# adamnelsonarcher/BB-OCR

Hardware: AMD Instinct MI355X
Metric: book-page images/sec end-to-end (detect+recognize) @1280x960 (higher is better)
Workload: dtype fp16

## Files before the change

bb-ocr_amd/csrc/conv_mfma.hip:

```cpp
#include "common.h"
#include "kernels.h"
#include <type_traits>
#include <utility>

template <int EL, int MF, bool ADDUP = false>
__device__ __forceinline__ void conv_epilogue(const ConvArgs& a, f32x4 (&acc)[MF][4], int n, int nt, int oy0, int ox0, int wm, int wn, int fpr,
                                              int lane, int BN, int sub = 1, int sph = 0, int spw = 0) {
    const int g = lane >> 4, pl = lane & 15;
    const int cout0 = nt * BN + wn * 64 + g * 8;
    if (a.tail) {
        const float* tw = a.tail;
        const typename El<EL>::v8 w1f = *(const typename El<EL>::v8*)(a.tail_frag + lane * 8);
        float cb[8], b1r[4], w2a[4], w2b[4];
#pragma unroll
        for (int i = 0; i < 8; ++i) cb[i] = a.bias[(g & 1) * 8 + i];
#pragma unroll
        for (int r = 0; r < 4; ++r) { b1r[r] = tw[4 * g + r]; w2a[r] = tw[16 + 4 * g + r]; w2b[r] = tw[32 + 4 * g + r]; }
        const float b20 = tw[48], b21 = tw[49];
#pragma unroll
        for (int f = 0; f < MF; ++f) {
            const int F = wm * MF + f;
            const int fr = F / fpr, fc = F - fr * fpr;
            const int oy = (oy0 + fr) * sub + sph, ox = (ox0 + fc * 16 + pl) * sub + spw;
            u32x4 bb;
#pragma unroll
            for (int j = 0; j < 2; ++j) {
                const float x0 = fmaxf(acc[f][j][0] + cb[j * 4 + 0], 0.f), x1 = fmaxf(acc[f][j][1] + cb[j * 4 + 1], 0.f);
                const float x2 = fmaxf(acc[f][j][2] + cb[j * 4 + 2], 0.f), x3 = fmaxf(acc[f][j][3] + cb[j * 4 + 3], 0.f);
// ... 62 lines not shown
            pack_runs(v, lo, hi);
            uint16_t* op = (uint16_t*)base + row + (size_t)x * cs + cout0 + coff;
            *(u32x4*)(op) = lo;
            if (run1) *(u32x4*)(op + 32) = hi;
        }
    };
    auto split_hi_lo = [&](const float (&v)[16], float (&vh)[16], float (&vl)[16]) {
#pragma unroll
        for (int i = 0; i < 16; ++i) {
            vh[i] = El<EL>::to_f32(El<EL>::from_f32(v[i]));
            vl[i] = (v[i] - vh[i]) * SPLIT_LO_SCALE;
        }
    };
    auto store_frag = [&](void* base, size_t row, int cs, int xb, int xlim, bool row_ok, const float (&v)[16], bool f32) {
        if (a.split_off) {
            float vh[16], vl[16];
            split_hi_lo(v, vh, vl);
            store_frag_at(base, row, cs, xb, xlim, row_ok, vh, false, 0);
            store_frag_at(base, row, cs, xb, xlim, row_ok, vl, false, a.split_off);
            return;
        }
        store_frag_at(base, row, cs, xb, xlim, row_ok, v, f32, 0);
    };
    if constexpr (ADDUP) {
        struct Gather { u32x4 q[8]; f32x2_t w[4]; };
        const int hw = a.up_H * a.up_W, LH = a.up_H >> 1, LW = a.up_W >> 1;
        const float rhw = 1.f / (float)hw, rw = 1.f / (float)a.up_W;
        auto issue = [&](int f, Gather& G) {
            int p = ox0 + (wm * MF + f) * 16 + pl;
            p = p < a.OW ? p : a.OW - 1;
            int ni = (int)((float)p * rhw);
            int rem = p - ni * hw;
            if (rem < 0) { --ni; rem += hw; } else if (rem >= hw) { ++ni; rem -= hw; }
            int yy = (int)((float)rem * rw);
            int xx = rem - yy * a.up_W;
            if (xx < 0) { --yy; xx += a.up_W; } else if (xx >= a.up_W) { ++yy; xx -= a.up_W; }
            float sy = ((float)yy + 0.5f) * 0.5f - 0.5f, sx = ((float)xx + 0.5f) * 0.5f - 0.5f;
            sy = sy < 0.f ? 0.f : sy;
            sx = sx < 0.f ? 0.f : sx;
            const int y0 = (int)sy, x0 = (int)sx;
            const int y1 = y0 + (y0 < LH - 1 ? 1 : 0), x1 = x0 + (x0 < LW - 1 ? 1 : 0);
            const float ly = sy - (float)y0, lx = sx - (float)x0, hy = 1.f - ly, hx = 1.f - lx;
            G.w[0] = (f32x2_t){hy * hx, hy * hx}; G.w[1] = (f32x2_t){hy * lx, hy * lx};
            G.w[2] = (f32x2_t){ly * hx, ly * hx}; G.w[3] = (f32x2_t){ly * lx, ly * lx};
            const uint16_t* zb = a.addup + (size_t)ni * LH * LW * a.up_cs + cout0;
            const uint16_t* z00 = zb + ((size_t)y0 * LW + x0) * a.up_cs;
            const uint16_t* z01 = zb + ((size_t)y0 * LW + x1) * a.up_cs;
// ... 1066 lines not shown
    const size_t smem = 18 * 2048 + 2 * 324 * 64 + 256;
    static LdsOptIn attr;
    if (hipError_t e = lds_opt_in(attr, (const void*)conv3x3_up4_kernel<EL>, smem); e != hipSuccess) return e;
    const int grid = ntiles < 2 * ncu ? ntiles : 2 * ncu;
    hipLaunchKernelGGL(conv3x3_up4_kernel<EL>, dim3(grid), dim3(256), smem, s, a);
    return hipGetLastError();
}

hipError_t launch_up4_fused(const ConvPlan& p1, const ConvPlan& p3, ConvArgs a, hipStream_t s) {
    if (p1.KH != 1 || p1.Cin != 128 || p1.Cout != 64 || p1.BN != 64 || p3.KH != 3 || p3.Cin != 64 || p3.Cout_pad != 64 || p3.BN != 64 ||
        p1.el != p3.el || p1.split || p3.split || a.in0_cs != 128 || a.up_cs != 64 || !a.addup || !a.zero || a.cout_store > 32 || (a.up_H & 1) || (a.up_W & 1) ||
        a.up_H != a.H || a.up_W != a.W)
        return hipErrorNotSupported;
    a.KH = a.KW = 3; a.pad_h = a.pad_w = 1; a.dil = 1; a.sub = 1;
    a.OH = a.H; a.OW = a.W; a.TH = a.TW = 16;
    a.tiles_x = (a.OW + 15) / 16; a.tiles_y = (a.OH + 15) / 16; a.ntiles_n = 1; a.nchunks = 2; a.ntaps = 9;
    a.aux_w = p1.d_w; a.aux_b = p1.d_b;
    a.wpk = p3.d_w; a.bias = p3.d_b;
    a.acc_scale = 1.f;
    if ((long long)a.N * a.tiles_x * a.tiles_y > 0x7fffffffLL) return hipErrorNotSupported;
    return p3.el ? launch_up4_el<1>(a, s) : launch_up4_el<0>(a, s);
}

template <int EL, int WM, int WN, int MF, int RING, bool ADDUP>
__global__ void __launch_bounds__(WM * WN * 64, (WM * WN == 8 ? 1 : 2)) conv1x1_dma_kernel(const ConvArgs a) {
    constexpr int NW = WM * WN, NT = NW * 64, BN = WN * 64;
    static_assert(NW == 4 || NW == 8, "wave w gathers 16 / NW of the 16-pixel blocks of the activation tile");
    constexpr int WBUF = BN * 64, WPIECES = WBUF / 16, WPT = WPIECES / NT;
    constexpr int NPX = WM * MF * 16, NPB = NPX / 64, PBUF = NPX * 64, SLOT = WBUF + PBUF;
    constexpr int PBW = NPB / (NW / 4);
    static_assert(WPIECES % NT == 0 && NPX == 256 && NPB % (NW / 4) == 0 && RING >= 3, "uniform DMA issue");
    extern __shared__ __attribute__((aligned(16))) unsigned char smem[];
    const int tid = threadIdx.x;
    const int lane = tid & 63;
    const int wave = __builtin_amdgcn_readfirstlane(tid >> 6);
    const int wm = wave / WN, wn = wave % WN;
    const size_t kg8 = ((lane & 3) ^ (((lane >> 4) & 1) * 2)) * 8;
    const int pb0 = wave * PBW;
    int bid = xcd_remap(blockIdx.x, gridDim.x);
    const int nt = bid % a.ntiles_n;
    const int tile = bid / a.ntiles_n;
    const int px0 = tile * NPX;
    const int nk = a.nchunks;
    int pix[PBW];
#pragma unroll
    for (int i = 0; i < PBW; ++i) {
        const int p = px0 + (pb0 + i) * 16 + (lane >> 2);
// ... 36 lines not shown
        }
        const unsigned char* sb = smem + slot * SLOT;
        typename El<EL>::v8 af[4], bq[MF];
#pragma unroll
        for (int j = 0; j < 4; ++j) af[j] = *(const typename El<EL>::v8*)(sb + lane_w_off + j * 1024);
#pragma unroll
        for (int f = 0; f < MF; ++f) bq[f] = *(const typename El<EL>::v8*)(sb + lane_p_off + f * 1024);
        if ((ks * 32 < a.C0) ? a.relu_in0 : a.relu_in1) {
            const s16x8 z = {0, 0, 0, 0, 0, 0, 0, 0};
#pragma unroll
            for (int f = 0; f < MF; ++f) bq[f] = __builtin_bit_cast(typename El<EL>::v8, __builtin_elementwise_max(__builtin_bit_cast(s16x8, bq[f]), z));
        }
#pragma unroll
        for (int f = 0; f < MF; ++f)
#pragma unroll
            for (int j = 0; j < 4; ++j) acc[f][j] = El<EL>::mfma(af[j], bq[f], acc[f][j]);
        if (ahead) asm volatile("s_waitcnt vmcnt(%0) lgkmcnt(0)\n\ts_barrier" ::"n"((RING - 2) * (WPT + PBW)) : "memory");
        else asm volatile("s_waitcnt vmcnt(0) lgkmcnt(0)\n\ts_barrier" ::: "memory");
        slot = slot + 1 == RING ? 0 : slot + 1;
    }
    conv_epilogue<EL, MF, ADDUP>(a, acc, 0, nt, 0, px0, wm, wn, 16, lane, BN);
}

template <int EL, int WM, int WN, int MF, bool ADDUP>
static hipError_t launch_dma1x1_k(const ConvArgs& a, long long grid, hipStream_t s, ConvRoute* route, bool dry) {
    constexpr int RING = 3, NPX = WM * MF * 16;
    auto k = conv1x1_dma_kernel<EL, WM, WN, MF, RING, ADDUP>;
    const size_t smem = (size_t)RING * ((size_t)WN * 64 * 64 + (size_t)NPX * 64);
    constexpr int id = ADDUP ? CONV_ROUTE_DMA1X1_ADDUP : (WN == 1 ? CONV_ROUTE_DMA1X1_64 : (WN == 2 ? CONV_ROUTE_DMA1X1_128 : CONV_ROUTE_DMA1X1_256));
    if (ConvRoute* r = route_fill(route, id, a, EL, WM, WN, MF, grid, smem)) { r->ring = RING; r->addup = ADDUP; r->ks = 1; }
    if (dry) return hipSuccess;
    static LdsOptIn attr;
    if (hipError_t e = lds_opt_in(attr, (const void*)k, smem); e != hipSuccess) return e;
    hipLaunchKernelGGL(k, dim3((int)grid), dim3(WM * WN * 64), smem, s, a);
    return hipGetLastError();
}

template <int EL, int WM, int WN, int MF>
static hipError_t launch_dma1x1(ConvArgs a, hipStream_t s, ConvRoute* route, bool dry) {
    constexpr int NPX = WM * MF * 16;
    const long long total = (long long)a.N * a.H * a.W;
    if (total > 0x7fffffffLL) return hipErrorInvalidValue;
    a.N = 1; a.OH = 1; a.OW = (int)total; a.TH = 1; a.TW = NPX; a.tiles_y = 1;
    a.tiles_x = (int)((total + NPX - 1) / NPX);
    const long long grid = (long long)a.tiles_x * a.ntiles_n;
    if (grid > 0x7fffffffLL) return hipErrorInvalidValue;
    return a.addup ? launch_dma1x1_k<EL, WM, WN, MF, true>(a, grid, s, route, dry) : launch_dma1x1_k<EL, WM, WN, MF, false>(a, grid, s, route, dry);
}

static inline int cdiv(int a, int b) { return (a + b - 1) / b; }

size_t conv_packed_elems(const ConvPlan& p) {
    return (size_t)p.Cout_pad * p.Cin_pad * p.KH * p.KW;
}

void pack_conv_weights(const ConvPlan& p, const float* w, uint16_t* out) {
    const int BN = p.BN, ntn = p.Cout_pad / BN, nch = p.Cin_pad / 32, ntaps = p.KH * p.KW, nfr = BN / 16;
    size_t o = 0;
    for (int nt = 0; nt < ntn; ++nt)
        for (int c = 0; c < nch; ++c)
            for (int tap = 0; tap < ntaps; ++tap)
                for (int fr = 0; fr < nfr; ++fr) {
                    const int wn = fr >> 2, nf = fr & 3;
                    for (int l = 0; l < 64; ++l) {
                        const int row = l & 15;
                        const int cout = nt * BN + wn * 64 + (nf >> 1) * 32 + (row >> 2) * 8 + (nf & 1) * 4 + (row & 3);
                        for (int j = 0; j < 8; ++j) {
                            const int cin = c * 32 + 8 * (l >> 4) + j;
                            float v = 0.f;
                            if (cout < p.Cout && cin < p.Cin) v = w[((size_t)cout * p.Cin + cin) * ntaps + tap];
// ... 141 lines not shown
            if (pit > max_piter || (size_t)ring * BN * 64 + (size_t)2 * np * 64 > 160 * 1024) continue;
            if (a.ntaps >= 3 ? (a.ntaps - 1) / nparts < 1 : nparts > 1) continue;
            if (a.pool_mode && (BN == 128 ? 8 : 4) % (2 * (tw / 16)) != 0) continue;
            const long long tiles = (long long)cdiv(a.OH, th) * cdiv(a.OW, tw);
            const long long cost = tiles * ((long long)BM * a.ntaps + 2LL * np);
            if (best < 0 || cost < best) { best = cost; a.TH = th; a.TW = tw; a.PH = ph; a.PW = pw; a.NP = np; }
        }
        if (best < 0) return hipErrorInvalidValue;
    }
    a.tiles_x = cdiv(a.OW, a.TW);
    a.tiles_y = cdiv(a.OH, a.TH);
    a.ntiles_n = p.Cout_pad / BN;
    a.nchunks = p.Cin_pad / 32;
    if (a.C0 + a.C1 != p.Cin_pad || (a.C0 & 31) || (a.C1 & 31)) return hipErrorInvalidValue;
    if ((a.in0_cs & 7) || (a.C1 && (a.in1_cs & 7)) || (a.out_cs & (a.out_f32 ? 3 : 7)) || (a.cout_store & 15)) return hipErrorInvalidValue;
    a.wpk = p.d_w;
    a.bias = p.d_b;
    const long long grid_ll = (long long)a.N * a.tiles_x * a.tiles_y * a.ntiles_n;
    if (grid_ll <= 0 || grid_ll > 0x7fffffffLL) return hipErrorInvalidValue;
    const int grid = (int)grid_ll;
    if (a.addup && !(p.KH == 1 && p.KW == 1 && a.zero && !a.pool_mode && !a.out_f32 && !a.tail && a.cout_store % 64 == 0 &&
                     a.cout_store == p.Cout_pad))
        return hipErrorInvalidValue;
    if (p.KH == 1 && p.KW == 1 && p.pad_h == 0 && p.pad_w == 0 && a.zero && !a.pool_mode)
        return BN == 256 ? launch_dma1x1<EL, 2, 4, 8>(a, s, route, dry) : (BN == 128 ? launch_dma1x1<EL, 2, 2, 8>(a, s, route, dry) : launch_dma1x1<EL, 4, 1, 4>(a, s, route, dry));
    if (dma2x2)
        return BN == 128 ? launch_dma_one<EL, 2, 2, 8, 6, 4, 384, false, 4, 0, 2>(a, grid, s, CONV_ROUTE_DMA2X2_128, route, dry)
                         : launch_dma_one<EL, 4, 1, 4, 6, 3, 384, false, 4, 0, 2>(a, grid, s, CONV_ROUTE_DMA2X2_64, route, dry);
    if (p.KH == 3 && p.KW == 3 && p.dil == 1 && p.pad_h == 1 && p.pad_w == 1 && a.zero) {
        const int npb = cdiv(a.PH * a.PW, 64);
        if (npb == 6 || npb == 7) {
            a.NP = npb * 64;
            return BN == 128 ? launch_dma<EL, 2, 2, 8>(a, npb, grid, s, route, dry) : launch_dma<EL, 4, 1, 4>(a, npb, grid, s, route, dry);
        }
    }
    if (a.c11_w || a.addup || a.post_w) return hipErrorNotSupported;
    const int piter = cdiv(a.NP / 16, NWV);
    if (BN == 128) return piter <= 4 ? launch_cfg<EL, 2, 2, 8, 4>(a, grid, s, route, dry) : (piter <= 8 ? launch_cfg<EL, 2, 2, 8, 8>(a, grid, s, route, dry) : launch_cfg<EL, 2, 2, 8, 16>(a, grid, s, route, dry));
    if (BN == 64) return piter <= 4 ? launch_cfg<EL, 4, 1, 4, 4>(a, grid, s, route, dry) : (piter <= 8 ? launch_cfg<EL, 4, 1, 4, 8>(a, grid, s, route, dry) : launch_cfg<EL, 4, 1, 4, 16>(a, grid, s, route, dry));
    return hipErrorInvalidValue;
}

hipError_t launch_conv(const ConvPlan& p, ConvArgs a, hipStream_t s, ConvRoute* route, bool dry) {
    if (route) *route = ConvRoute{};
    a.acc_scale = p.acc_scale;
    hipError_t e = hipErrorInvalidValue;
// ... 6 lines not shown
```

bb-ocr_amd/csrc/ctx.h:

```cpp
#pragma once
#include "../../include/bbocr.h"

#include <algorithm>
#include <atomic>
#include <chrono>
#include <condition_variable>
#include <cmath>
#include <cstring>
#include <functional>
#include <map>
#include <memory>
#include <mutex>
#include <string>
#include <thread>
#include <unordered_map>
#include <vector>

#include "boxpost.h"
#include "hostpool.h"
#include "common.h"
#include "kernels.h"


using clk = std::chrono::steady_clock;
// ... 96 lines not shown
inline void check_page(const DevPage& g, unsigned allowed = PAGE_ANY) {
    if (!g.p) fail(BBOCR_ERR_ARG, "null device pointer");
    if (g.H < 1 || g.W < 1) fail(BBOCR_ERR_ARG, "bad image shape");
    if ((long long)g.H * g.W >= (1LL << 30)) fail(BBOCR_ERR_ARG, "image too large");
    if (g.layout < PAGE_GRAY || g.layout > PAGE_YCC3 || !(allowed & page_set(g.layout))) fail(BBOCR_ERR_ARG, "layout must be one of the BBOCR_PAGE_* taken here");
    if (g.pitch < (long long)g.W * page_px_bytes(g.layout)) fail(BBOCR_ERR_ARG, "row pitch smaller than a row");
}

struct SideLane {
    std::mutex mu;
    hipStream_t stream = nullptr;
};



struct WeightView {
    bool craft_loaded = false;
    uint16_t* c11_wf = nullptr;
    float* c11_b = nullptr;
    float* c11_w32 = nullptr;
    float* cls6_w32 = nullptr;
    ConvPlan conv1_2, conv2_1, conv2_2, conv3_1, conv3_2, conv3_3, conv4_1, conv4_2, conv4_3, conv5_1, conv5_2, fc6, fc7;
    ConvPlan up1a, up1b, up2b, up3b, up4b, cls0, cls2, cls4;
    ConvPlan up2y, up2s, up3y, up3s, up4y, up4s;
    float* cls_tail = nullptr;
    uint16_t* cls_tail_frag = nullptr;
    uint16_t* up4y_post = nullptr;
    bool crnn_loaded = false;
    float* r0_wb = nullptr;
    uint16_t* r0_afrag = nullptr;
    ConvPlan r1, r2, r3, r4, r5, r6, xproj[2], lin[2], pred;
    uint16_t* pred_wide = nullptr;
    float* pred_wide_b = nullptr;
    uint16_t* whh[2] = {nullptr, nullptr};
    float whh_scale[2] = {1.f, 1.f};
    struct Q8Layer { int8_t* w = nullptr; float* scale = nullptr; float* bias = nullptr; };
    Q8Layer q_ih[2], q_hh[2], q_lin[2], q_pred;
    void* zero_page = nullptr;
};

struct bbocr_ctx : WeightView {
    bbocr_config cfg{};
    int cfg_beam_wide = 0;
    bbocr_ctx* root = nullptr;
    std::vector<bbocr_ctx*> slots;
    std::mutex pool_mu;
// ... 171 lines not shown
    RecPart part;
};

constexpr int REC_GAP = 4;
constexpr int REC_STAGES = 8;

template <typename T> inline T* upload(bbocr_ctx* c, const std::vector<T>& v) {
    void* d = nullptr;
    HIPCHK(hipMalloc(&d, v.size() * sizeof(T)));
    c->owned.push_back(d);
    c->owned_bytes.push_back(v.size() * sizeof(T));
    HIPCHK(hipMemcpy(d, v.data(), v.size() * sizeof(T), hipMemcpyHostToDevice));
    return (T*)d;
}

ConvPlan make_plan(int Cin, int Cout, int KH, int KW, int pad, int dil, int el = 0, int bn = 0);
void upload_plan(bbocr_ctx* c, ConvPlan& p, const std::vector<float>& w, const std::vector<float>& b);
void free_weights(bbocr_ctx* c);
size_t weights_blob_bytes(const bbocr_ctx* c);
void weights_export(bbocr_ctx* c, void* dev_dst, size_t bytes);
void weights_import(bbocr_ctx* c, const void* dev_src, size_t bytes);
void load_craft(bbocr_ctx* c, const TensorMap& tm);
void load_crnn(bbocr_ctx* c, const TensorMap& tm);
ConvArgs conv_args(const ConvPlan& p, const Act& a0, const Act* a1 = nullptr, const Act* addup = nullptr);
hipError_t launch_conv_profiled(bbocr_ctx* c, const ConvPlan& p, ConvArgs a, bool may_decline = false);
void run_conv(bbocr_ctx* c, const ConvPlan& p, const Act& a0, bool relu0, const Act* a1, bool relu1, bool relu_out, void* out, int out_cs, int cout_store, bool out_f32, const Act* addup = nullptr);
hipError_t launch_seq_proj_profiled(bbocr_ctx* c, const ConvPlan& p, const uint16_t* x, size_t rows_pad, uint16_t* out);
void prof_collect(bbocr_ctx* c);
Act conv_act(bbocr_ctx* c, const ConvPlan& p, const Act& a0, bool relu0, const Act* a1, bool relu1, bool relu_out, int store);
Act conv_pool_act(bbocr_ctx* c, const ConvPlan& p, const Act& a0, bool relu0, bool relu_out, int store, int mode, bool pool_relu, Act* full, const RgbSource* rgb = nullptr);
Act pool_act(bbocr_ctx* c, const Act& a, int kh, int kw, int sh, int sw, int ph, int pw, bool relu_in);
void craft_up_stage(bbocr_ctx* c, const ConvPlan& py, const ConvPlan& ps, const Act& y, const Act& skip, uint16_t* z, uint16_t* out);
bool craft_up3b_post(bbocr_ctx* c, const Act& u3a, uint16_t* u3b, uint16_t* z);
bool craft_up4(bbocr_ctx* c, const Act& s1, const uint16_t* z, uint16_t* u4b);
void craft_cls_tail(bbocr_ctx* c, const Act& c2, float* heat);
struct ExactConvRow {
    const char* name;
    ConvPlan bbocr_ctx::* plan;
    bool relu_out;
    int store;
    int pool_mode;
    bool pool_relu;
    bool keep_full;
};
int craft_exact_rows();
const ExactConvRow& craft_exact_row(int row);
Act craft_exact_conv(bbocr_ctx* c, int row, const Act& in, Act* full = nullptr);
Act craft_exact_conv1_1(bbocr_ctx* c, const uint8_t* rgb, int nb, int Himg, int Wimg, int H32, int W32);
Act craft_exact_relu(bbocr_ctx* c, const Act& a);
Act craft_exact_upcat(bbocr_ctx* c, const Act& y, const Act& skip);
Act craft_exact_pool5(bbocr_ctx* c, const Act& s4);
void craft_exact_cls_tail(bbocr_ctx* c, const Act& c3, float* heat);
DetDims det_dims(int H, int W, int canvas, double mag);
void detect_impl(bbocr_ctx* c, const uint8_t* rgb, int B, int H, int W, const bbocr_params& p, float* heat, const std::function<void(int, int)>& after_sub = nullptr);
DetPlan det_plan(bbocr_ctx* c, int B, int H, int W, const bbocr_params& p, bool overlapped);
// ... 198 lines not shown
```

bb-ocr_amd/csrc/detector.cpp:

```cpp
#include "ctx.h"

static hipEvent_t prof_event(bbocr_ctx* c) {
    hipEvent_t e;
    if (!c->prof_pool.empty()) { e = c->prof_pool.back(); c->prof_pool.pop_back(); }
    else HIPCHK(hipEventCreate(&e));
    return e;
}

template <typename F> static hipError_t profiled(bbocr_ctx* c, double flops, F&& launch) {
    if (c->profiling == 0 || (c->profiling == 1 && c->prof_group != 0)) return launch();
    bbocr_ctx::ProfRec r{prof_event(c), prof_event(c), flops, c->prof_group};
    HIPCHK(hipEventRecord(r.e0, c->cur));
    const hipError_t e = launch();
    HIPCHK(hipEventRecord(r.e1, c->cur));
    if (e == hipSuccess) c->prof_recs.push_back(r);
    else prof_release(c, r);
    return e;
}

hipError_t launch_conv_profiled(bbocr_ctx* c, const ConvPlan& p, ConvArgs a, bool may_decline) {
    a.zero = c->zero_page;
    const int OH = a.H + 2 * p.pad_h - (p.KH - 1) * p.dil, OW = a.W + 2 * p.pad_w - (p.KW - 1) * p.dil;
    double flops = 2.0 * a.N * OH * OW * (double)p.Cout * (p.split ? p.Cin / 3 : p.Cin) * p.KH * p.KW;
    if (a.c11_w) flops += 2.0 * a.N * a.H * a.W * 64.0 * 27.0;
    if (a.tail) flops += 2.0 * a.N * OH * OW * (16.0 * 16.0 + 16.0 * 2.0);
    if (a.post_w) flops += 2.0 * a.N * OH * OW * 64.0 * 64.0;
    const hipError_t e = profiled(c, flops, [&] { return launch_conv(p, a, c->cur); });
    if (may_decline && e == hipErrorNotSupported) return e;
    HIPCHK(e);
    return hipSuccess;
}

hipError_t launch_seq_proj_profiled(bbocr_ctx* c, const ConvPlan& p, const uint16_t* x, size_t rows_pad, uint16_t* out) {
    const double flops = 2.0 * (double)rows_pad * (double)p.Cout * p.Cin;
    const hipError_t e = profiled(c, flops, [&] { return launch_seq_proj(p, x, rows_pad, out, c->cur); });
    if (e != hipErrorNotSupported) HIPCHK(e);
    return e;
}

ConvArgs conv_args(const ConvPlan& p, const Act& a0, const Act* a1, const Act* addup) {
    ConvArgs a{};
    a.in0 = a0.p; a.C0 = a0.C; a.in0_cs = a0.C;
    a.N = a0.N; a.H = a0.H; a.W = a0.W;
    if (p.split) {
        if (a1 || (a0.C & 63)) fail(BBOCR_ERR_INTERNAL, "split-fp16 conv: one pair tensor with a multiple of 32 logical channels expected");
        a.in1 = a0.p; a.C1 = a0.C / 2; a.in1_cs = a0.C;
    } else if (a1) {
        a.in1 = a1->p; a.C1 = a1->C; a.in1_cs = a1->C;
    }
    if (addup) { a.addup = addup->p; a.up_H = a0.H; a.up_W = a0.W; a.up_cs = addup->C; }
    return a;
}

void run_conv(bbocr_ctx* c, const ConvPlan& p, const Act& a0, bool relu0, const Act* a1, bool relu1, bool relu_out, void* out,
                     int out_cs, int cout_store, bool out_f32, const Act* addup) {
    if (c->arena.dry) return;
    ConvArgs a = conv_args(p, a0, a1, addup);
    a.relu_in0 = relu0; a.relu_in1 = p.split ? relu0 : relu1; a.relu_out = relu_out; a.out_f32 = out_f32;
    a.out = out; a.out_cs = out_cs; a.cout_store = cout_store;
    if (p.split && !out_f32) a.split_off = cout_store;
    (void)launch_conv_profiled(c, p, a);
}

void prof_collect(bbocr_ctx* c) {
    bbocr_ctx* root = c->root;
    std::lock_guard<std::mutex> lk(root->pool_mu);
    for (auto& r : c->prof_recs) {
        float ms = 0.f;
        if (hipEventElapsedTime(&ms, r.e0, r.e1) == hipSuccess) {
            root->prof_ms[r.group] += ms;
            root->prof_flops[r.group] += r.flops;
            root->prof_launches[r.group] += 1;
        }
        prof_release(c, r);
    }
    c->prof_recs.clear();
}

static Act arena_act(bbocr_ctx* c, int N, int H, int W, int C) { return Act{c->arena.alloc<uint16_t>((size_t)N * H * W * C), N, H, W, C}; }

// ... 16 lines not shown
    ConvArgs a = conv_args(p, a0);
    a.relu_in0 = relu0; a.relu_in1 = relu0; a.relu_out = relu_out; a.out_f32 = 0;
    a.out = full ? (void*)full->p : nullptr; a.out_cs = cs; a.cout_store = store;
    if (p.split) a.split_off = store;
    a.pool_mode = mode; a.pool_relu = pool_relu; a.store_full = full != nullptr; a.pool_cs = cs; a.pool_out = o.p;
    if (rgb) { a.in0 = (const uint16_t*)rgb->rgb; a.c11_w = c->c11_wf; a.c11_b = c->c11_b; a.rgb_H = rgb->Himg; a.rgb_W = rgb->Wimg; }
    (void)launch_conv_profiled(c, p, a);
    return o;
}

Act pool_act(bbocr_ctx* c, const Act& a, int kh, int kw, int sh, int sw, int ph, int pw, bool relu_in) {
    const int OH = (a.H + 2 * ph - kh) / sh + 1, OW = (a.W + 2 * pw - kw) / sw + 1;
    Act o = arena_act(c, a.N, OH, OW, a.C);
    if (!c->arena.dry) HIPCHK(launch_maxpool(a.p, o.p, a.N, a.H, a.W, a.C, kh, kw, sh, sw, ph, pw, relu_in, c->cur));
    return o;
}


void craft_up_stage(bbocr_ctx* c, const ConvPlan& py, const ConvPlan& ps, const Act& y, const Act& skip, uint16_t* z, uint16_t* out) {
    const int cout = ps.Cout;
    const Act zz{z, y.N, y.H, y.W, cout};
    run_conv(c, py, y, false, nullptr, false, false, z, cout, cout, false);
    run_conv(c, ps, skip, false, nullptr, false, true, out, cout, cout, false, &zz);
}

bool craft_up3b_post(bbocr_ctx* c, const Act& u3a, uint16_t* u3b, uint16_t* z) {
    if (c->arena.dry) return false;
    if (c->up4y_post && !c->up3b.split) {
        ConvArgs a = conv_args(c->up3b, u3a);
        a.relu_out = 1; a.out = z; a.out_cs = 64; a.cout_store = 64; a.post_w = c->up4y_post;
        if (launch_conv_profiled(c, c->up3b, a, true) == hipSuccess) return true;
    }
    const Act b{u3b, u3a.N, u3a.H, u3a.W, 64};
    run_conv(c, c->up3b, u3a, false, nullptr, false, true, u3b, 64, 64, false);
    run_conv(c, c->up4y, b, false, nullptr, false, false, z, 64, 64, false);
    return false;
}

bool craft_up4(bbocr_ctx* c, const Act& s1, const uint16_t* z, uint16_t* u4b) {
    const Act zz{(uint16_t*)z, s1.N, s1.H / 2, s1.W / 2, 64};
    if (!c->arena.dry) {
        ConvArgs a = conv_args(c->up4s, s1, nullptr, &zz);
        a.relu_out = 1; a.out = u4b; a.out_cs = 32; a.cout_store = 32;
        a.zero = c->zero_page;
        const hipError_t e = profiled(c, 2.0 * a.N * a.H * a.W * (128.0 * 64.0 + 64.0 * 32.0 * 9.0), [&] { return launch_up4_fused(c->up4s, c->up4b, a, c->cur); });
        if (e == hipSuccess) return true;
// ... 9 lines not shown
    if (c->arena.dry) return;
    ConvArgs a = conv_args(c->cls4, c2);
    a.relu_out = 1; a.out = heat; a.out_cs = 16; a.cout_store = 16; a.tail = c->cls_tail; a.tail_frag = c->cls_tail_frag;
    (void)launch_conv_profiled(c, c->cls4, a);
}

static void craft_forward(bbocr_ctx* c, const uint8_t* rgb, int nb, int Himg, int Wimg, int H32, int W32, float* heat) {
    c->prof_group = 0;
    const Act canvas{nullptr, nb, H32, W32, 64};
    const RgbSource src{rgb, Himg, Wimg};
    Act p1 = conv_pool_act(c, c->conv1_2, canvas, false, true, 64, 1, false, nullptr, &src);
    Act a3 = conv_act(c, c->conv2_1, p1, false, nullptr, false, true, 128);
    Act s1;
    Act p2 = conv_pool_act(c, c->conv2_2, a3, false, false, 128, 1, true, &s1);
    Act a5 = conv_act(c, c->conv3_1, p2, false, nullptr, false, true, 256);
    Act s2 = conv_act(c, c->conv3_2, a5, false, nullptr, false, false, 256);
    Act p3 = conv_pool_act(c, c->conv3_3, s2, true, true, 256, 1, false, nullptr);
    Act a8 = conv_act(c, c->conv4_1, p3, false, nullptr, false, true, 512);
    Act s3 = conv_act(c, c->conv4_2, a8, false, nullptr, false, false, 512);
    Act p4 = conv_pool_act(c, c->conv4_3, s3, true, true, 512, 1, false, nullptr);
    Act a11 = conv_act(c, c->conv5_1, p4, false, nullptr, false, true, 512);
    Act s4 = conv_act(c, c->conv5_2, a11, false, nullptr, false, false, 512);
    Act p5 = pool_act(c, s4, 3, 3, 1, 1, 1, 1, false);
    Act f6 = conv_act(c, c->fc6, p5, false, nullptr, false, false, 1024);
    Act f7 = conv_act(c, c->fc7, f6, false, nullptr, false, false, 1024);
    Act u1a = conv_act(c, c->up1a, f7, false, &s4, false, true, 512);
    Act u1b = conv_act(c, c->up1b, u1a, false, nullptr, false, true, 256);
    Act z2 = arena_act(c, u1b.N, u1b.H, u1b.W, 256), u2a = arena_act(c, s3.N, s3.H, s3.W, 256);
    craft_up_stage(c, c->up2y, c->up2s, u1b, s3, z2.p, u2a.p);
    Act u2b = conv_act(c, c->up2b, u2a, false, nullptr, false, true, 128);
    Act z3 = arena_act(c, u2b.N, u2b.H, u2b.W, 128), u3a = arena_act(c, s2.N, s2.H, s2.W, 128);
    craft_up_stage(c, c->up3y, c->up3s, u2b, s2, z3.p, u3a.p);
    Act u3b = arena_act(c, u3a.N, u3a.H, u3a.W, 64), z4 = arena_act(c, u3a.N, u3a.H, u3a.W, 64);
    (void)craft_up3b_post(c, u3a, u3b.p, z4.p);
    Act u4b = arena_act(c, s1.N, s1.H, s1.W, 32);
    (void)craft_up4(c, s1, z4.p, u4b.p);
    Act c1 = conv_act(c, c->cls0, u4b, false, nullptr, false, true, 32);
    Act c2 = conv_act(c, c->cls2, c1, false, nullptr, false, true, 32);
    craft_cls_tail(c, c2, heat);
}

static Act pair_act(bbocr_ctx* c, int N, int H, int W, int C) { return arena_act(c, N, H, W, 2 * C); }

static const ExactConvRow kExactConvs[] = {
    {"conv1_2", &bbocr_ctx::conv1_2, true, 64, 1, false, false},
    {"conv2_1", &bbocr_ctx::conv2_1, true, 128, 0, false, false},
    {"conv2_2", &bbocr_ctx::conv2_2, false, 128, 1, true, true},
    {"conv3_1", &bbocr_ctx::conv3_1, true, 256, 0, false, false},
    {"conv3_2", &bbocr_ctx::conv3_2, false, 256, 0, false, false},
// ... 277 lines not shown
```

bb-ocr_amd/csrc/kernels.h:

```cpp
#pragma once
#include <hip/hip_runtime.h>
#include <stdint.h>
#include <vector>

struct ConvArgs {
    const uint16_t* in0;
    const uint16_t* in1;
    const uint16_t* wpk;
    const float* bias;
    void* out;
    int C0, C1;
    int in0_cs, in1_cs;
    int N, H, W, OH, OW;
    int KH, KW, pad_h, pad_w, dil;
    int TH, TW, tiles_x, tiles_y, ntiles_n;
    int PH, PW, NP;
    int relu_in0, relu_in1, relu_out, out_f32;
    int out_cs, cout_store;
    int nchunks, ntaps;
    int pool_mode, pool_relu, store_full, pool_cs;
    void* pool_out;
    const uint16_t* aux_w;
    const float* tail;
    const uint16_t* tail_frag;
    const uint16_t* post_w;
    int sub;
    int stack;
    const void* zero;
    const uint16_t* addup;
    int up_H, up_W, up_cs;
    const uint16_t* c11_w;
    const float* c11_b;
    int rgb_H, rgb_W;
    const float* aux_b;
    float acc_scale;
    int lean;
    int split_off;
};

struct ConvPlan {
    int Cin = 0, Cout = 0;
    int Cin_pad = 0, Cout_pad = 0;
    int KH = 1, KW = 1, pad_h = 0, pad_w = 0, dil = 1;
    int BN = 64;
    int el = 0;
    float acc_scale = 1.f;
    int split = 0;
    uint16_t* d_w = nullptr;
    float* d_b = nullptr;
};

enum ConvRouteId : int {
    CONV_ROUTE_NONE = 0,
    CONV_ROUTE_GEN64_P4, CONV_ROUTE_GEN64_P8, CONV_ROUTE_GEN64_P16, CONV_ROUTE_GEN128_P4, CONV_ROUTE_GEN128_P8, CONV_ROUTE_GEN128_P16,
    CONV_ROUTE_DMA64_FUSE1, CONV_ROUTE_DMA64_POSTW,
    CONV_ROUTE_RESW_POOL64, CONV_ROUTE_RESW_1CH, CONV_ROUTE_RESW_2CH,
    CONV_ROUTE_DMA64_324_NF2, CONV_ROUTE_DMA64_324, CONV_ROUTE_DMA64_384, CONV_ROUTE_DMA64_448,
    CONV_ROUTE_DMA128_384, CONV_ROUTE_DMA128_448,
    CONV_ROUTE_DMA2X2_64, CONV_ROUTE_DMA2X2_128,
    CONV_ROUTE_DMA1X1_64, CONV_ROUTE_DMA1X1_128, CONV_ROUTE_DMA1X1_256, CONV_ROUTE_DMA1X1_ADDUP,
// ... 325 lines not shown
```

bb-ocr_amd/csrc/weights.cpp:

```cpp
#include "ctx.h"
#include <limits>


static void fold_conv(const TensorMap& tm, const std::string& conv, const std::string& bn, int Cout, int Cin, int K, std::vector<float>& w,
                      std::vector<float>& b) {
    const size_t per = (size_t)Cin * K;
    const float* cw = tm.get(conv + ".weight", (size_t)Cout * per);
    const float* cb = tm.get(conv + ".bias", (size_t)Cout, false);
    w.assign(cw, cw + (size_t)Cout * per);
    b.assign(Cout, 0.f);
    if (cb) std::copy(cb, cb + Cout, b.begin());
    if (!bn.empty()) {
        const float* g = tm.get(bn + ".weight", Cout);
        const float* be = tm.get(bn + ".bias", Cout);
        const float* mu = tm.get(bn + ".running_mean", Cout);
        const float* var = tm.get(bn + ".running_var", Cout);
        for (int o = 0; o < Cout; ++o) {
            const float sc = g[o] / std::sqrt(var[o] + 1e-5f);
            for (size_t i = 0; i < per; ++i) w[(size_t)o * per + i] *= sc;
            b[o] = (b[o] - mu[o]) * sc + be[o];
        }
    }
}

// ... 77 lines not shown
    c->owned.clear();
    c->owned_bytes.clear();
    c->craft_loaded = c->crnn_loaded = false;
}

namespace {
struct BlobHeader { unsigned long long magic; int precision, nblocks; unsigned long long bytes; int craft, crnn; unsigned long long layout_hash; int rec_quant; int rec_classes; int pad[4]; };
static_assert(sizeof(BlobHeader) == 64, "blob header");
constexpr unsigned long long BLOB_MAGIC = 0x62626f6372776231ULL;
unsigned long long layout_hash(const bbocr_ctx* c) {
    unsigned long long h = 1469598103934665603ULL;
    for (size_t b : c->owned_bytes)
        for (int i = 0; i < 8; ++i) { h ^= (unsigned long long)((b >> (8 * i)) & 0xff); h *= 1099511628211ULL; }
    return h;
}
std::vector<float*> blob_scalars(bbocr_ctx* c) {
    std::vector<float*> v;
    for (ConvPlan* p : {&c->r1, &c->r2, &c->r3, &c->r4, &c->r5, &c->r6, &c->xproj[0], &c->xproj[1], &c->lin[0], &c->lin[1], &c->pred}) v.push_back(&p->acc_scale);
    v.push_back(&c->whh_scale[0]);
    v.push_back(&c->whh_scale[1]);
    for (ConvPlan* p : {&c->conv1_2, &c->conv2_1, &c->conv2_2, &c->conv3_1, &c->conv3_2, &c->conv3_3, &c->conv4_1, &c->conv4_2, &c->conv4_3, &c->conv5_1,
                        &c->conv5_2, &c->fc6, &c->fc7, &c->up1a, &c->up1b, &c->up2s, &c->up2b, &c->up3s, &c->up3b, &c->up4s, &c->up4b, &c->cls0, &c->cls2, &c->cls4})
        v.push_back(&p->acc_scale);
    return v;
}
}

size_t weights_blob_bytes(const bbocr_ctx* c) {
    size_t n = sizeof(BlobHeader);
    for (size_t b : c->owned_bytes) n += align_up(b, 256);
    return n + 256;
}

void weights_export(bbocr_ctx* c, void* dev_dst, size_t bytes) {
    if (!c->craft_loaded && !c->crnn_loaded) fail(BBOCR_ERR_STATE, "no weights loaded");
    if (bytes != weights_blob_bytes(c)) fail(BBOCR_ERR_ARG, "weight blob: wrong size");
    BlobHeader h{};
    h.magic = BLOB_MAGIC; h.precision = c->cfg.precision; h.nblocks = (int)c->owned.size(); h.bytes = bytes;
    h.craft = c->craft_loaded; h.crnn = c->crnn_loaded; h.layout_hash = layout_hash(c); h.rec_quant = c->cfg.rec_quant;
    h.rec_classes = (c->crnn_loaded && rec_classes(c) != kRecClassesDefault) ? rec_classes(c) : 0;
    char* d = (char*)dev_dst;
    HIPCHK(hipMemcpyAsync(d, &h, sizeof(h), hipMemcpyHostToDevice, c->stream));
    size_t off = sizeof(h);
    for (size_t i = 0; i < c->owned.size(); ++i) {
        HIPCHK(hipMemcpyAsync(d + off, c->owned[i], c->owned_bytes[i], hipMemcpyDeviceToDevice, c->stream));
        off += align_up(c->owned_bytes[i], 256);
// ... 60 lines not shown
    L(c->up2b, "upconv2.conv.3", "upconv2.conv.4", 256, 128, 3, 1, 1);
    L(c->up3s, "upconv3.conv.0", "upconv3.conv.1", 384, 128, 1, 0, 1);
    L(c->up3b, "upconv3.conv.3", "upconv3.conv.4", 128, 64, 3, 1, 1);
    L(c->up4s, "upconv4.conv.0", "upconv4.conv.1", 192, 64, 1, 0, 1);
    L(c->up4b, "upconv4.conv.3", "upconv4.conv.4", 64, 32, 3, 1, 1);
    L(c->cls0, "conv_cls.0", "", 32, 32, 3, 1, 1);
    L(c->cls2, "conv_cls.2", "", 32, 32, 3, 1, 1);
    L(c->cls4, "conv_cls.4", "", 32, 16, 3, 1, 1);
    {
        const float* w1 = tm.get("conv_cls.6.weight", 256);
        const float* b1 = tm.get("conv_cls.6.bias", 16);
        const float* w2 = tm.get("conv_cls.8.weight", 32);
        const float* b2 = tm.get("conv_cls.8.bias", 2);
        std::vector<float> t(50);
        std::copy(b1, b1 + 16, t.begin());
        std::copy(w2, w2 + 32, t.begin() + 16);
        std::copy(b2, b2 + 2, t.begin() + 48);
        c->cls_tail = upload(c, t);
        c->cls6_w32 = upload(c, std::vector<float>(w1, w1 + 256));
    }
    c->craft_loaded = true;
}

void load_craft(bbocr_ctx* c, const TensorMap& tm) {
    if (det_split(c)) { load_craft_exact(c, tm); return; }
    {
        std::vector<float> w, b;
        fold_conv(tm, "basenet.slice1.0", "basenet.slice1.1", 64, 3, 9, w, b);
        std::vector<uint16_t> pk(4 * 64 * 8);
        pack_conv1_1_weights_fused(w.data(), pk.data(), det_el(c));
        c->c11_wf = upload(c, pk);
        c->c11_b = upload(c, b);
    }
    load_layer(c, tm, c->conv1_2, "basenet.slice1.3", "basenet.slice1.4", 64, 64, 3, 1, 1, det_el(c));
    load_layer(c, tm, c->conv2_1, "basenet.slice1.7", "basenet.slice1.8", 64, 128, 3, 1, 1, det_el(c));
    load_layer(c, tm, c->conv2_2, "basenet.slice1.10", "basenet.slice1.11", 128, 128, 3, 1, 1, det_el(c));
    load_layer(c, tm, c->conv3_1, "basenet.slice2.14", "basenet.slice2.15", 128, 256, 3, 1, 1, det_el(c));
    load_layer(c, tm, c->conv3_2, "basenet.slice2.17", "basenet.slice2.18", 256, 256, 3, 1, 1, det_el(c));
    load_layer(c, tm, c->conv3_3, "basenet.slice3.20", "basenet.slice3.21", 256, 256, 3, 1, 1, det_el(c));
    load_layer(c, tm, c->conv4_1, "basenet.slice3.24", "basenet.slice3.25", 256, 512, 3, 1, 1, det_el(c));
    load_layer(c, tm, c->conv4_2, "basenet.slice3.27", "basenet.slice3.28", 512, 512, 3, 1, 1, det_el(c));
    load_layer(c, tm, c->conv4_3, "basenet.slice4.30", "basenet.slice4.31", 512, 512, 3, 1, 1, det_el(c));
    load_layer(c, tm, c->conv5_1, "basenet.slice4.34", "basenet.slice4.35", 512, 512, 3, 1, 1, det_el(c));
    load_layer(c, tm, c->conv5_2, "basenet.slice4.37", "basenet.slice4.38", 512, 512, 3, 1, 1, det_el(c));
    load_layer(c, tm, c->fc6, "basenet.slice5.1", "", 512, 1024, 3, 6, 6, det_el(c));
    load_layer(c, tm, c->fc7, "basenet.slice5.2", "", 1024, 1024, 1, 0, 1, det_el(c), false, 256);
    load_layer(c, tm, c->up1a, "upconv1.conv.0", "upconv1.conv.1", 1536, 512, 1, 0, 1, det_el(c), false, 256);
    load_layer(c, tm, c->up1b, "upconv1.conv.3", "upconv1.conv.4", 512, 256, 3, 1, 1, det_el(c));
    load_split_1x1(c, tm, c->up2y, c->up2s, "upconv2.conv.0", "upconv2.conv.1", 256, 512, 256);
    load_layer(c, tm, c->up2b, "upconv2.conv.3", "upconv2.conv.4", 256, 128, 3, 1, 1, det_el(c));
    load_split_1x1(c, tm, c->up3y, c->up3s, "upconv3.conv.0", "upconv3.conv.1", 128, 256, 128);
    load_layer(c, tm, c->up3b, "upconv3.conv.3", "upconv3.conv.4", 128, 64, 3, 1, 1, det_el(c));
    {
        std::vector<float> wy;
        load_split_1x1(c, tm, c->up4y, c->up4s, "upconv4.conv.0", "upconv4.conv.1", 64, 128, 64, &wy);
        std::vector<uint16_t> pk(2 * 4 * 64 * 8);
        pack_post1x1_weights(wy.data(), pk.data(), det_el(c));
        c->up4y_post = upload(c, pk);
    }
    load_layer(c, tm, c->up4b, "upconv4.conv.3", "upconv4.conv.4", 64, 32, 3, 1, 1, det_el(c));
    load_layer(c, tm, c->cls0, "conv_cls.0", "", 32, 32, 3, 1, 1, det_el(c));
    load_layer(c, tm, c->cls2, "conv_cls.2", "", 32, 32, 3, 1, 1, det_el(c));
    load_layer(c, tm, c->cls4, "conv_cls.4", "", 32, 16, 3, 1, 1, det_el(c));
    {
        const float* w1 = tm.get("conv_cls.6.weight", 256);
        const float* b1 = tm.get("conv_cls.6.bias", 16);
        const float* w2 = tm.get("conv_cls.8.weight", 32);
        const float* b2 = tm.get("conv_cls.8.bias", 2);
        std::vector<float> t(50);
        std::copy(b1, b1 + 16, t.begin());
// ... 166 lines not shown
```

Before: 990.7.

## Fold fc6, fc7 and upconv1 1x1 into one dilated conv plus skip 1x1

Since fc6 (3x3 dilated, 512->1024), fc7 (1x1, 1024->1024) and the first upconv1 1x1 (1536->512) are linear with no activation between them, the host precomposes their weights into a single 3x3 dilated conv 512->512 plus a 1x1 on the skip input. It adds a same-resolution addend epilogue variant for the 1x1 DMA kernel to sum the two partial results. This removes two large convolutions and their intermediate 1024-channel activations. The fp16 output may differ numerically because the fold reassociates the products, and the weights are composed in double precision on the host at load time.

```diff
diff --git a/bb-ocr_amd/csrc/conv_mfma.hip b/bb-ocr_amd/csrc/conv_mfma.hip
--- a/bb-ocr_amd/csrc/conv_mfma.hip
+++ b/bb-ocr_amd/csrc/conv_mfma.hip
@@ -3,7 +3,7 @@
 #include <type_traits>
 #include <utility>
 
-template <int EL, int MF, bool ADDUP = false>
+template <int EL, int MF, int ADDUP = 0>
 __device__ __forceinline__ void conv_epilogue(const ConvArgs& a, f32x4 (&acc)[MF][4], int n, int nt, int oy0, int ox0, int wm, int wn, int fpr,
                                               int lane, int BN, int sub = 1, int sph = 0, int spw = 0) {
     const int g = lane >> 4, pl = lane & 15;
@@ -112,7 +112,38 @@
         }
         store_frag_at(base, row, cs, xb, xlim, row_ok, v, f32, 0);
     };
-    if constexpr (ADDUP) {
+    if constexpr (ADDUP == 2) {
+        struct Addend { u32x4 q[2]; };
+        auto issue = [&](int f, Addend& G) {
+            int p = ox0 + (wm * MF + f) * 16 + pl;
+            p = p < a.OW ? p : a.OW - 1;
+            const uint16_t* zb = a.addup + (size_t)p * a.up_cs + cout0;
+            G.q[0] = *(const u32x4*)zb;
+            G.q[1] = *(const u32x4*)(zb + 32);
+        };
+        Addend G[2];
+        issue(0, G[0]);
+#pragma unroll
+        for (int f = 0; f < MF; ++f) {
+            if (f + 1 < MF) issue(f + 1, G[(f + 1) & 1]);
+            __builtin_amdgcn_sched_barrier(0);
+            const Addend& C = G[f & 1];
+            float v[16];
+#pragma unroll
+            for (int h = 0; h < 2; ++h)
+#pragma unroll
+                for (int i = 0; i < 4; ++i) {
+                    const f32x2_t t = El<EL>::unpack2(C.q[h][i]);
+                    const int k = h * 8 + i * 2;
+                    float x0 = acc[f][k >> 2][k & 3] + bs[k] + t[0], x1 = acc[f][(k + 1) >> 2][(k + 1) & 3] + bs[k + 1] + t[1];
+                    if (a.relu_out) { x0 = fmaxf(x0, 0.f); x1 = fmaxf(x1, 0.f); }
+                    v[k] = x0; v[k + 1] = x1;
+                }
+            store_frag(a.out, 0, a.out_cs, ox0 + (wm * MF + f) * 16, a.OW, true, v, false);
+        }
+        return;
+    }
+    if constexpr (ADDUP == 1) {
         struct Gather { u32x4 q[8]; f32x2_t w[4]; };
         const int hw = a.up_H * a.up_W, LH = a.up_H >> 1, LW = a.up_W >> 1;
         const float rhw = 1.f / (float)hw, rw = 1.f / (float)a.up_W;
@@ -1225,7 +1256,7 @@
     return p3.el ? launch_up4_el<1>(a, s) : launch_up4_el<0>(a, s);
 }
 
-template <int EL, int WM, int WN, int MF, int RING, bool ADDUP>
+template <int EL, int WM, int WN, int MF, int RING, int ADDUP>
 __global__ void __launch_bounds__(WM * WN * 64, (WM * WN == 8 ? 1 : 2)) conv1x1_dma_kernel(const ConvArgs a) {
     constexpr int NW = WM * WN, NT = NW * 64, BN = WN * 64;
     static_assert(NW == 4 || NW == 8, "wave w gathers 16 / NW of the 16-pixel blocks of the activation tile");
@@ -1308,7 +1339,7 @@
     conv_epilogue<EL, MF, ADDUP>(a, acc, 0, nt, 0, px0, wm, wn, 16, lane, BN);
 }
 
-template <int EL, int WM, int WN, int MF, bool ADDUP>
+template <int EL, int WM, int WN, int MF, int ADDUP>
 static hipError_t launch_dma1x1_k(const ConvArgs& a, long long grid, hipStream_t s, ConvRoute* route, bool dry) {
     constexpr int RING = 3, NPX = WM * MF * 16;
     auto k = conv1x1_dma_kernel<EL, WM, WN, MF, RING, ADDUP>;
@@ -1331,7 +1362,8 @@
     a.tiles_x = (int)((total + NPX - 1) / NPX);
     const long long grid = (long long)a.tiles_x * a.ntiles_n;
     if (grid > 0x7fffffffLL) return hipErrorInvalidValue;
-    return a.addup ? launch_dma1x1_k<EL, WM, WN, MF, true>(a, grid, s, route, dry) : launch_dma1x1_k<EL, WM, WN, MF, false>(a, grid, s, route, dry);
+    if (a.addup && a.add_same) return launch_dma1x1_k<EL, WM, WN, MF, 2>(a, grid, s, route, dry);
+    return a.addup ? launch_dma1x1_k<EL, WM, WN, MF, 1>(a, grid, s, route, dry) : launch_dma1x1_k<EL, WM, WN, MF, 0>(a, grid, s, route, dry);
 }
 
 static inline int cdiv(int a, int b) { return (a + b - 1) / b; }
@@ -1519,6 +1551,7 @@
     if (a.addup && !(p.KH == 1 && p.KW == 1 && a.zero && !a.pool_mode && !a.out_f32 && !a.tail && a.cout_store % 64 == 0 &&
                      a.cout_store == p.Cout_pad))
         return hipErrorInvalidValue;
+    if (a.add_same && !(a.addup && a.up_H == a.H && a.up_W == a.W && a.up_cs == a.cout_store)) return hipErrorInvalidValue;
     if (p.KH == 1 && p.KW == 1 && p.pad_h == 0 && p.pad_w == 0 && a.zero && !a.pool_mode)
         return BN == 256 ? launch_dma1x1<EL, 2, 4, 8>(a, s, route, dry) : (BN == 128 ? launch_dma1x1<EL, 2, 2, 8>(a, s, route, dry) : launch_dma1x1<EL, 4, 1, 4>(a, s, route, dry));
     if (dma2x2)
diff --git a/bb-ocr_amd/csrc/ctx.h b/bb-ocr_amd/csrc/ctx.h
--- a/bb-ocr_amd/csrc/ctx.h
+++ b/bb-ocr_amd/csrc/ctx.h
@@ -142,6 +142,7 @@
     float* cls6_w32 = nullptr;
     ConvPlan conv1_2, conv2_1, conv2_2, conv3_1, conv3_2, conv3_3, conv4_1, conv4_2, conv4_3, conv5_1, conv5_2, fc6, fc7;
     ConvPlan up1a, up1b, up2b, up3b, up4b, cls0, cls2, cls4;
+    ConvPlan fcfold, up1s;
     ConvPlan up2y, up2s, up3y, up3s, up4y, up4s;
     float* cls_tail = nullptr;
     uint16_t* cls_tail_frag = nullptr;
@@ -359,15 +360,16 @@
 void weights_import(bbocr_ctx* c, const void* dev_src, size_t bytes);
 void load_craft(bbocr_ctx* c, const TensorMap& tm);
 void load_crnn(bbocr_ctx* c, const TensorMap& tm);
-ConvArgs conv_args(const ConvPlan& p, const Act& a0, const Act* a1 = nullptr, const Act* addup = nullptr);
+ConvArgs conv_args(const ConvPlan& p, const Act& a0, const Act* a1 = nullptr, const Act* addup = nullptr, const Act* addsame = nullptr);
 hipError_t launch_conv_profiled(bbocr_ctx* c, const ConvPlan& p, ConvArgs a, bool may_decline = false);
-void run_conv(bbocr_ctx* c, const ConvPlan& p, const Act& a0, bool relu0, const Act* a1, bool relu1, bool relu_out, void* out, int out_cs, int cout_store, bool out_f32, const Act* addup = nullptr);
+void run_conv(bbocr_ctx* c, const ConvPlan& p, const Act& a0, bool relu0, const Act* a1, bool relu1, bool relu_out, void* out, int out_cs, int cout_store, bool out_f32, const Act* addup = nullptr, const Act* addsame = nullptr);
 hipError_t launch_seq_proj_profiled(bbocr_ctx* c, const ConvPlan& p, const uint16_t* x, size_t rows_pad, uint16_t* out);
 void prof_collect(bbocr_ctx* c);
 Act conv_act(bbocr_ctx* c, const ConvPlan& p, const Act& a0, bool relu0, const Act* a1, bool relu1, bool relu_out, int store);
 Act conv_pool_act(bbocr_ctx* c, const ConvPlan& p, const Act& a0, bool relu0, bool relu_out, int store, int mode, bool pool_relu, Act* full, const RgbSource* rgb = nullptr);
 Act pool_act(bbocr_ctx* c, const Act& a, int kh, int kw, int sh, int sw, int ph, int pw, bool relu_in);
 void craft_up_stage(bbocr_ctx* c, const ConvPlan& py, const ConvPlan& ps, const Act& y, const Act& skip, uint16_t* z, uint16_t* out);
+void craft_fc_stage(bbocr_ctx* c, const Act& p5, const Act& s4, uint16_t* z, uint16_t* out);
 bool craft_up3b_post(bbocr_ctx* c, const Act& u3a, uint16_t* u3b, uint16_t* z);
 bool craft_up4(bbocr_ctx* c, const Act& s1, const uint16_t* z, uint16_t* u4b);
 void craft_cls_tail(bbocr_ctx* c, const Act& c2, float* heat);
diff --git a/bb-ocr_amd/csrc/detector.cpp b/bb-ocr_amd/csrc/detector.cpp
--- a/bb-ocr_amd/csrc/detector.cpp
+++ b/bb-ocr_amd/csrc/detector.cpp
@@ -38,7 +38,7 @@
     return e;
 }
 
-ConvArgs conv_args(const ConvPlan& p, const Act& a0, const Act* a1, const Act* addup) {
+ConvArgs conv_args(const ConvPlan& p, const Act& a0, const Act* a1, const Act* addup, const Act* addsame) {
     ConvArgs a{};
     a.in0 = a0.p; a.C0 = a0.C; a.in0_cs = a0.C;
     a.N = a0.N; a.H = a0.H; a.W = a0.W;
@@ -49,13 +49,17 @@
         a.in1 = a1->p; a.C1 = a1->C; a.in1_cs = a1->C;
     }
     if (addup) { a.addup = addup->p; a.up_H = a0.H; a.up_W = a0.W; a.up_cs = addup->C; }
+    if (addsame) {
+        if (addup || addsame->N != a0.N) fail(BBOCR_ERR_INTERNAL, "conv: one addend, of the output's own page count");
+        a.addup = addsame->p; a.up_H = addsame->H; a.up_W = addsame->W; a.up_cs = addsame->C; a.add_same = 1;
+    }
     return a;
 }
 
 void run_conv(bbocr_ctx* c, const ConvPlan& p, const Act& a0, bool relu0, const Act* a1, bool relu1, bool relu_out, void* out,
-                     int out_cs, int cout_store, bool out_f32, const Act* addup) {
+                     int out_cs, int cout_store, bool out_f32, const Act* addup, const Act* addsame) {
     if (c->arena.dry) return;
-    ConvArgs a = conv_args(p, a0, a1, addup);
+    ConvArgs a = conv_args(p, a0, a1, addup, addsame);
     a.relu_in0 = relu0; a.relu_in1 = p.split ? relu0 : relu1; a.relu_out = relu_out; a.out_f32 = out_f32;
     a.out = out; a.out_cs = out_cs; a.cout_store = cout_store;
     if (p.split && !out_f32) a.split_off = cout_store;
@@ -118,6 +122,13 @@
     const Act zz{z, y.N, y.H, y.W, cout};
     run_conv(c, py, y, false, nullptr, false, false, z, cout, cout, false);
     run_conv(c, ps, skip, false, nullptr, false, true, out, cout, cout, false, &zz);
+}
+
+void craft_fc_stage(bbocr_ctx* c, const Act& p5, const Act& s4, uint16_t* z, uint16_t* out) {
+    const int cout = c->up1s.Cout;
+    const Act zz{z, p5.N, p5.H, p5.W, cout};
+    run_conv(c, c->fcfold, p5, false, nullptr, false, false, z, cout, cout, false);
+    run_conv(c, c->up1s, s4, false, nullptr, false, true, out, cout, cout, false, nullptr, &zz);
 }
 
 bool craft_up3b_post(bbocr_ctx* c, const Act& u3a, uint16_t* u3b, uint16_t* z) {
@@ -173,9 +184,8 @@
     Act a11 = conv_act(c, c->conv5_1, p4, false, nullptr, false, true, 512);
     Act s4 = conv_act(c, c->conv5_2, a11, false, nullptr, false, false, 512);
     Act p5 = pool_act(c, s4, 3, 3, 1, 1, 1, 1, false);
-    Act f6 = conv_act(c, c->fc6, p5, false, nullptr, false, false, 1024);
-    Act f7 = conv_act(c, c->fc7, f6, false, nullptr, false, false, 1024);
-    Act u1a = conv_act(c, c->up1a, f7, false, &s4, false, true, 512);
+    Act z1 = arena_act(c, s4.N, s4.H, s4.W, 512), u1a = arena_act(c, s4.N, s4.H, s4.W, 512);
+    craft_fc_stage(c, p5, s4, z1.p, u1a.p);
     Act u1b = conv_act(c, c->up1b, u1a, false, nullptr, false, true, 256);
     Act z2 = arena_act(c, u1b.N, u1b.H, u1b.W, 256), u2a = arena_act(c, s3.N, s3.H, s3.W, 256);
     craft_up_stage(c, c->up2y, c->up2s, u1b, s3, z2.p, u2a.p);
diff --git a/bb-ocr_amd/csrc/fc_fold.h b/bb-ocr_amd/csrc/fc_fold.h
--- /dev/null
+++ b/bb-ocr_amd/csrc/fc_fold.h
@@ -0,0 +1,68 @@
+#pragma once
+#include <algorithm>
+#include <cstddef>
+#include <vector>
+
+#include "hostpool.h"
+
+struct FcFoldDims {
+    int Cin, M6, M7, Cout, Cs, taps;
+};
+
+namespace fc_fold_detail {
+constexpr int RB = 4, CB = 8;
+inline int pad_rows(int M) { return (M + RB - 1) / RB * RB; }
+
+template <typename T, typename F>
+void gemm(int M, int K, int N, const double* At, const T* B, double* C, F&& parallel) {
+    const int Mp = pad_rows(M);
+    parallel((N + CB - 1) / CB, [&, M, K, N, Mp](int t) {
+        const int c0 = t * CB, nc = std::min(CB, N - c0);
+        std::vector<double> strip((size_t)K * CB, 0.0);
+        for (int k = 0; k < K; ++k)
+            for (int j = 0; j < nc; ++j) strip[(size_t)k * CB + j] = (double)B[(size_t)k * N + c0 + j];
+        for (int o0 = 0; o0 < M; o0 += RB) {
+            double acc[RB][CB] = {};
+            for (int k = 0; k < K; ++k) {
+                const double* a = At + (size_t)k * Mp + o0;
+                const double* w = strip.data() + (size_t)k * CB;
+                for (int r = 0; r < RB; ++r)
+                    for (int j = 0; j < CB; ++j) acc[r][j] += a[r] * w[j];
+            }
+            for (int r = 0; r < RB && o0 + r < M; ++r)
+                for (int j = 0; j < nc; ++j) C[(size_t)(o0 + r) * N + c0 + j] = acc[r][j];
+        }
+    });
+}
+}
+
+template <typename T>
+void fc_fold(const FcFoldDims& d, const T* w6, const T* b6, const T* w7, const T* b7, const T* wu, const T* bu, std::vector<T>& wc, std::vector<T>& ws,
+             std::vector<T>& bp, HostPool* pool = nullptr) {
+    using namespace fc_fold_detail;
+    const size_t per = (size_t)d.Cin * d.taps, cu = (size_t)d.M7 + d.Cs;
+    const int Mp = pad_rows(d.Cout);
+    auto parallel = [&](int n, const std::function<void(int)>& fn) {
+        if (pool) pool->parallel_for(n, fn);
+        else for (int i = 0; i < n; ++i) fn(i);
+    };
+    std::vector<double> Yt((size_t)d.M7 * Mp, 0.0), A((size_t)d.Cout * d.M6, 0.0);
+    for (int o = 0; o < d.Cout; ++o)
+        for (int m = 0; m < d.M7; ++m) Yt[(size_t)m * Mp + o] = (double)wu[o * cu + m];
+    gemm(d.Cout, d.M7, d.M6, Yt.data(), w7, A.data(), parallel);
+    ws.assign((size_t)d.Cout * d.Cs, T(0));
+    bp.assign(d.Cout, T(0));
+    for (int o = 0; o < d.Cout; ++o) {
+        double s = (double)bu[o];
+        for (int m = 0; m < d.M7; ++m) s += (double)wu[o * cu + m] * (double)b7[m];
+        for (int k = 0; k < d.M6; ++k) s += A[(size_t)o * d.M6 + k] * (double)b6[k];
+        bp[o] = (T)s;
+        for (int i = 0; i < d.Cs; ++i) ws[(size_t)o * d.Cs + i] = wu[o * cu + d.M7 + i];
+    }
+    std::vector<double> At((size_t)d.M6 * Mp, 0.0), C((size_t)d.Cout * per, 0.0);
+    for (int o = 0; o < d.Cout; ++o)
+        for (int k = 0; k < d.M6; ++k) At[(size_t)k * Mp + o] = A[(size_t)o * d.M6 + k];
+    gemm(d.Cout, d.M6, (int)per, At.data(), w6, C.data(), parallel);
+    wc.resize(C.size());
+    for (size_t i = 0; i < C.size(); ++i) wc[i] = (T)C[i];
+}
diff --git a/bb-ocr_amd/csrc/kernels.h b/bb-ocr_amd/csrc/kernels.h
--- a/bb-ocr_amd/csrc/kernels.h
+++ b/bb-ocr_amd/csrc/kernels.h
@@ -36,6 +36,7 @@
     float acc_scale;
     int lean;
     int split_off;
+    int add_same;
 };
 
 struct ConvPlan {
diff --git a/bb-ocr_amd/csrc/weights.cpp b/bb-ocr_amd/csrc/weights.cpp
--- a/bb-ocr_amd/csrc/weights.cpp
+++ b/bb-ocr_amd/csrc/weights.cpp
@@ -1,4 +1,5 @@
 #include "ctx.h"
+#include "fc_fold.h"
 #include <limits>
 
 
@@ -123,6 +124,7 @@
     for (ConvPlan* p : {&c->conv1_2, &c->conv2_1, &c->conv2_2, &c->conv3_1, &c->conv3_2, &c->conv3_3, &c->conv4_1, &c->conv4_2, &c->conv4_3, &c->conv5_1,
                         &c->conv5_2, &c->fc6, &c->fc7, &c->up1a, &c->up1b, &c->up2s, &c->up2b, &c->up3s, &c->up3b, &c->up4s, &c->up4b, &c->cls0, &c->cls2, &c->cls4})
         v.push_back(&p->acc_scale);
+    for (ConvPlan* p : {&c->fcfold, &c->up1s}) v.push_back(&p->acc_scale);
     return v;
 }
 }
@@ -229,6 +231,28 @@
     c->craft_loaded = true;
 }
 
+static void load_fc_fold(bbocr_ctx* c, const TensorMap& tm) {
+    std::vector<float> wu, bu;
+    fold_conv(tm, "upconv1.conv.0", "upconv1.conv.1", 512, 1536, 1, wu, bu);
+    c->up1a = make_plan(1536, 512, 1, 1, 0, 1, det_el(c), 256);
+    upload_plan(c, c->up1a, wu, bu);
+    std::vector<float> w6, b6;
+    fold_conv(tm, "basenet.slice5.1", "", 1024, 512, 9, w6, b6);
+    c->fc6 = make_plan(512, 1024, 3, 3, 6, 6, det_el(c));
+    upload_plan(c, c->fc6, w6, b6);
+    const FcFoldDims d{512, 1024, 1024, 512, 512, 9};
+    std::vector<float> wc((size_t)d.Cout * d.Cin * d.taps, 0.f), ws((size_t)d.Cout * d.Cs, 0.f), bp(d.Cout, 0.f);
+    if (!tm.zeros) {
+        std::vector<float> w7, b7;
+        fold_conv(tm, "basenet.slice5.2", "", 1024, 1024, 1, w7, b7);
+        fc_fold(d, w6.data(), b6.data(), w7.data(), b7.data(), wu.data(), bu.data(), wc, ws, bp, &host_pool(c));
+    }
+    c->fcfold = make_plan(512, 512, 3, 3, 6, 6, det_el(c));
+    upload_plan(c, c->fcfold, wc, std::vector<float>(512, 0.f));
+    c->up1s = make_plan(512, 512, 1, 1, 0, 1, det_el(c));
+    upload_plan(c, c->up1s, ws, bp);
+}
+
 void load_craft(bbocr_ctx* c, const TensorMap& tm) {
     if (det_split(c)) { load_craft_exact(c, tm); return; }
     {
@@ -250,9 +274,7 @@
     load_layer(c, tm, c->conv4_3, "basenet.slice4.30", "basenet.slice4.31", 512, 512, 3, 1, 1, det_el(c));
     load_layer(c, tm, c->conv5_1, "basenet.slice4.34", "basenet.slice4.35", 512, 512, 3, 1, 1, det_el(c));
     load_layer(c, tm, c->conv5_2, "basenet.slice4.37", "basenet.slice4.38", 512, 512, 3, 1, 1, det_el(c));
-    load_layer(c, tm, c->fc6, "basenet.slice5.1", "", 512, 1024, 3, 6, 6, det_el(c));
-    load_layer(c, tm, c->fc7, "basenet.slice5.2", "", 1024, 1024, 1, 0, 1, det_el(c), false, 256);
-    load_layer(c, tm, c->up1a, "upconv1.conv.0", "upconv1.conv.1", 1536, 512, 1, 0, 1, det_el(c), false, 256);
+    load_fc_fold(c, tm);
     load_layer(c, tm, c->up1b, "upconv1.conv.3", "upconv1.conv.4", 512, 256, 3, 1, 1, det_el(c));
     load_split_1x1(c, tm, c->up2y, c->up2s, "upconv2.conv.0", "upconv2.conv.1", 256, 512, 256);
     load_layer(c, tm, c->up2b, "upconv2.conv.3", "upconv2.conv.4", 256, 128, 3, 1, 1, det_el(c));
```

Result: faster. 1027 (median of 6 runs) (+3.7%).
